# kisasexypantera94/hpfw

Hardware: AMD Instinct MI355X
Metric: hashprints/sec (index) + Hamming matches/sec (search), 30 s@44.1 kHz clips (higher is better)
Workload: dtype f32 (transforms, dB) + int8 digits / int64 sums (projection); 1 GPU; configs[1]: 1000 x 30 s synthetic 44.1 kHz PCM16 clips per GPU, hashprint extraction only (CQT + dB + projection + bit pack), inputs resident in HBM; clips_per_gpu=1000, hashprints_per_clip=2320, parallelism=clips sharded over 1 GPU(s), no collective on this path

## Files before the change

hpfw_amd/csrc/extract.hip:

```cpp
#include "handle.h"

int pass_clips(hpfw_gpu *h, const DevPlan *dp, int64_t n_clips)
{
    const hpfw::HostPlan &p = dp->hp;
    size_t per_clip = (size_t)121 * p.c * 4 + (size_t)64 * std::max(p.n_frames, 1) * 4;
    if (p.bluestein)
        per_clip += 2 * hpfw::bz_plane_bytes(dp->bz, 1) + (size_t)(p.kmax - p.kmin) * 8;
    else
        per_clip += (size_t)hpfw::z_floats_per_clip(p.hq, p.n2) * 4 + (size_t)p.n1 * p.q2w * 8;
    size_t work = 0;
    for (const hpfw::CqClassDev &cd : dp->cls) work = std::max(work, hpfw::cq_big_work_bytes(cd, 1));
    per_clip += work;
    const int64_t fit = std::max<int64_t>(1, (int64_t)(((size_t)24 << 30) / per_clip));
    const int64_t cap = std::min<int64_t>(h->batch, fit), n = std::max<int64_t>(n_clips, 1);
    const int64_t passes = (n + cap - 1) / cap;
    return (int)((n + passes - 1) / passes);
}

int ensure_ws(hpfw_gpu *h, const DevPlan *dp, int nb, int ns)
{
    const hpfw::HostPlan &p = dp->hp;
    size_t work = 0;
    for (const hpfw::CqClassDev &cd : dp->cls) work = std::max(work, hpfw::cq_big_work_bytes(cd, nb));
    if (work) {
        int rc = ensure(h->d_cqwork, work);
        if (rc) return rc;
    }
    const size_t planar = p.bluestein ? hpfw::bz_plane_bytes(dp->bz, nb) : 0;
    const size_t need[7] = {p.bluestein ? planar : (size_t)nb * hpfw::z_floats_per_clip(p.hq, p.n2) * 4,
                            p.bluestein ? (size_t)nb * (p.kmax - p.kmin) * 8 : (size_t)nb * p.n1 * p.q2w * 8,
                            (size_t)ns * 121 * p.c * 4, (size_t)ns * 64 * (size_t)std::max(p.n_frames, 1) * 4,
                            (size_t)ns * 121 * hpfw::kCqMaxWaves * 4,
                            0, planar};
    for (int i = 0; i < 7; ++i) {
        int rc = ensure(h->ws[i], need[i], h);
        if (rc) return rc;
    }
    return ensure(h->d_clipmax, (size_t)ns * 4, h);
}

namespace {
int ensure_side_streams(hpfw_gpu *h)
{
    if (h->cq_join[hpfw_gpu::kCqSide - 1]) return HPFW_OK;
    bool ok = h->cq_fork.create() == hipSuccess;
    for (int k = 0; k < hpfw_gpu::kCqSide && ok; ++k) ok = h->cq_side[k].create() == hipSuccess && h->cq_join[k].create() == hipSuccess;
    return ok ? HPFW_OK : fail(HPFW_E_HIP, "side streams");
}

class Fanout {
public:
    Fanout(hpfw_gpu *h, hipStream_t s) : h_(h), s_(s) {}
    Fanout(const Fanout &) = delete;
    Fanout &operator=(const Fanout &) = delete;
    ~Fanout()
    {
        for (int k = 0; k < hpfw_gpu::kCqSide; ++k) {
            if (!(used_ >> k & 1u)) continue;
            hipStream_t side = h_->cq_side[k].get();
            hipEvent_t join = h_->cq_join[k].get();
            if (report(h_, hipEventRecord(join, side), "side stream join") || report(h_, hipStreamWaitEvent(s_, join, 0), "side stream join"))
                (void)hipStreamSynchronize(side);
        }
    }
    int fork(int n)
    {
        int rc = ensure_side_streams(h_);
        if (rc) return rc;
        HIP_TRY(hipEventRecord(h_->cq_fork.get(), s_));
        for (int k = 0; k < n; ++k) HIP_TRY(hipStreamWaitEvent(h_->cq_side[k].get(), h_->cq_fork.get(), 0));
        return 0;
    }
    hipStream_t lane(int k)
    {
        if (k == 0) return s_;
        used_ |= 1u << (k - 1);
        return h_->cq_side[k - 1].get();
    }

private:
    hpfw_gpu *h_;
    hipStream_t s_;
    unsigned used_ = 0;
};

#if defined(HPFW_ROWS_SNAP) || defined(HPFW_ROWS_STAMPS)
hpfw::cf *g_rows_snap = nullptr;
#endif

int run_forward(hpfw_gpu *h, DevPlan *dp, const int16_t *d_pcm, int nb, hpfw::cf *x, hipStream_t s)
{
    const hpfw::HostPlan &p = dp->hp;
    float *yp = h->ws[0].as<float>();
    int rc;
    if (p.bluestein) {
        float *other = h->ws[6].as<float>();
        if (h->bz_chunk > 0 && nb >= 6 * h->bz_chunk) {
            const int lanes = h->fwd_streams;
            Fanout fan(h, s);
            if (lanes > 1 && (rc = fan.fork(lanes - 1))) return rc;
            const int64_t region = (int64_t)(hpfw::bz_plane_bytes(dp->bz, h->bz_chunk) / sizeof(float));
            int i = 0;
            for (int c0 = 0; c0 < nb; c0 += h->bz_chunk, ++i) {
                const int nc = std::min(nb - c0, h->bz_chunk);
                const int lane = i % lanes;
                hipStream_t st = fan.lane(lane);
                float *ya = yp + lane * region, *yb = other + lane * region;
                {
                    Timed t(h, K_COLS, st);
                    hpfw::launch_bz_cols_first(dp->bz, d_pcm + (int64_t)c0 * p.n, p.n, nc, ya, st);
                }
                {
                    Timed t(h, K_ROWS, st);
                    hpfw::launch_bz_rows_both(dp->rows, dp->bz, ya, nc, yb, st);
                }
                {
                    Timed t(h, K_COLS, st);
                    hpfw::launch_bz_cols_last(dp->bz, yb, nc, x + (int64_t)c0 * dp->cq.xclip, st);
                }
            }
            return check_launch("bz_chunks");
        }
        {
            Timed t(h, K_COLS, s);
            hpfw::launch_bz_cols_first(dp->bz, d_pcm, p.n, nb, yp, s);
        }
        if ((rc = check_launch("bz_cols"))) return rc;
        {
            Timed t(h, K_ROWS, s);
            hpfw::launch_bz_rows_both(dp->rows, dp->bz, yp, nb, other, s);
        }
        if ((rc = check_launch("bz_rows"))) return rc;
        {
            Timed t(h, K_COLS, s);
            hpfw::launch_bz_cols_last(dp->bz, other, nb, x, s);
        }
        return check_launch("bz_cols");
    }
    Timed span(h, K_FWD, s);
    hpfw::ColsQArgs cols = dp->cols;
    cols.variant = h->cols_variant;
    if (h->fwd_chunk > 0 && nb >= 6 * h->fwd_chunk) {
        const int lanes = h->fwd_streams;
        Fanout fan(h, s);
        if (lanes > 1 && (rc = fan.fork(lanes - 1))) return rc;
        const int64_t region = (int64_t)h->fwd_chunk * dp->rows_out.zclip;
        int i = 0;
        for (int c0 = 0; c0 < nb; c0 += h->fwd_chunk, ++i) {
            const int nc = std::min(nb - c0, h->fwd_chunk);
            const int lane = i % lanes;
            hipStream_t st = fan.lane(lane);
            float *zr = yp + lane * region;
            {
                Timed t(h, K_COLS, st);
                hpfw::launch_fwd_cols_q(cols, d_pcm + (int64_t)c0 * p.n, p.n, nc, zr, st);
            }
            {
                Timed t(h, K_ROWS, st);
                hpfw::launch_fwd_rows2(dp->rows, dp->rows_out, zr, nc, x + (int64_t)c0 * dp->rows_out.n1 * dp->rows_out.q2w, st);
            }
        }
        return check_launch("fwd_chunks");
    }
    {
        Timed t(h, K_COLS, s);
        hpfw::launch_fwd_cols_q(cols, d_pcm, p.n, nb, yp, s);
    }
    if ((rc = check_launch("fwd_cols"))) return rc;
    {
        Timed t(h, K_ROWS, s);
#if defined(HPFW_ROWS_SNAP)
        dp->rows.snap = g_rows_snap;
#endif
#if defined(HPFW_ROWS_STAMPS)
        dp->rows.stamps = reinterpret_cast<long long *>(g_rows_snap);
#endif
        hpfw::launch_fwd_rows2(dp->rows, dp->rows_out, yp, nb, x, s);
    }
    return check_launch("fwd_rows");
}
}

int run_front(hpfw_gpu *h, DevPlan *dp, const int16_t *d_pcm, int nb, int slot, bool finish_db, hipStream_t s)
{
    using hpfw::cf;
    const hpfw::HostPlan &p = dp->hp;
    cf *x = h->ws[1].as<cf>();
    float *mag = h->ws[2].as<float>() + (size_t)slot * 121 * p.c;
    float *mm = h->ws[4].as<float>() + (size_t)slot * 121 * hpfw::kCqMaxWaves;
    float *clipmax = h->d_clipmax.as<float>() + slot;
    int rc;
    if ((rc = run_forward(h, dp, d_pcm, nb, x, s))) return rc;
    {
        Timed t(h, K_CQ, s);
        int n_lds = 0;
        for (const hpfw::CqClassDev &cd : dp->cls) n_lds += cd.outer ? 0 : 1;
        const bool fork = h->cq_concurrent && n_lds > 1 && nb >= 4;
        Fanout fan(h, s);
        if (fork && (rc = fan.fork(hpfw_gpu::kCqSide))) return rc;
        int turn = 0;
        for (size_t ci = dp->cls.size(); ci-- > 0;) {
            const hpfw::CqClassDev &cd = dp->cls[ci];
            if (cd.outer) {
                hpfw::launch_cq_big_class(dp->cq, cd, x, nb, h->d_cqwork.as<cf>(), mag, mm, h->db_fast ? hpfw::kDbFast : hpfw::kDbSpec, s);
                continue;
            }
            const int lane = fork ? turn++ % (hpfw_gpu::kCqSide + 1) : 0;
            hpfw::launch_cq_class(dp->cq, cd, x, nb, mag, mm, h->db_fast ? hpfw::kDbFast : hpfw::kDbSpec, fan.lane(lane));
        }
        if ((rc = check_launch("cq_chirpz"))) return rc;
    }
    {
        Timed t(h, K_DB, s);
        hpfw::launch_clipmax(mm, clipmax, nb, s);
        if (finish_db) hpfw::launch_db_finish(mag, clipmax, nb, (int64_t)121 * p.c, s);
    }
    return check_launch("db");
}

namespace {
int run_back(hpfw_gpu *h, DevPlan *dp, const void *images, int n_shifts, int ns, uint64_t *d_hp, hipStream_t s)
{
    const hpfw::HostPlan &p = dp->hp;
    const float *sdb = h->ws[2].as<float>();
    int rc;
    if (h->projection) {
        {
            Timed t(h, K_PROJECT, s);
            hpfw::launch_hashprints_q(images, n_shifts, sdb, h->d_clipmax.as<float>(), ns, p.c, d_hp, nullptr, s);
        }
        return check_launch("project");
    }
    float *proj = h->ws[3].as<float>();
    {
        Timed t(h, K_PROJECT, s);
        hpfw::launch_project(h->d_fpack.as<float>(), sdb, h->d_clipmax.as<float>(), ns, p.c, proj, s);
    }
    if ((rc = check_launch("project"))) return rc;
    {
        Timed t(h, K_PACK, s);
        hpfw::launch_pack(proj, ns, p.n_frames, d_hp, s);
    }
    return check_launch("delta_pack");
}

constexpr int kBackBatch = 1024;

int check_filters(const hpfw_gpu *h) { return h->has_filters ? 0 : fail(HPFW_E_NOFILTERS, "no filters: call hpfw_gpu_set_filters or hpfw_gpu_learn_filters first"); }

int check_shifts(const int32_t *shifts, int n_shifts)
{
    if (!shifts || n_shifts < 1 || n_shifts > hpfw::kMaxShifts) return fail(HPFW_E_INVALID, "shifts: 1 to 64 values");
    for (int i = 0; i < n_shifts; ++i) {
        if (shifts[i] < -(hpfw::kBins - 1) || shifts[i] > hpfw::kBins - 1) return fail(HPFW_E_INVALID, "shifts: |s| <= 120");
        for (int j = 0; j < i; ++j)
            if (shifts[j] == shifts[i]) return fail(HPFW_E_INVALID, "shifts: values must be distinct");
    }
    return 0;
}

int shift_images(hpfw_gpu *h, const int32_t *shifts, int n_shifts, hipStream_t s)
{
    std::vector<int32_t> want(shifts, shifts + n_shifts);
    if (want == h->shift_images_of) return 0;
    h->shift_images_of.clear();
    int rc;
    if ((rc = ensure(h->d_shift_images, (size_t)n_shifts * hpfw::project_q_image_bytes()))) return rc;
    hpfw::ShiftList sl{n_shifts, {}};
    for (int i = 0; i < n_shifts; ++i) sl.s[i] = shifts[i];
    hpfw::launch_shift_filter_images(h->d_fq_image.get(), sl, h->d_shift_images.get(), s);
    if ((rc = check_launch("shift_filter_images"))) return rc;
    h->shift_images_of = std::move(want);
    return 0;
}

int check_transposed(hpfw_gpu *h, const int32_t *shifts, int n_shifts)
{
    int rc;
    if ((rc = check_shifts(shifts, n_shifts))) return rc;
    if (!h) return fail(HPFW_E_INVALID, "null handle");
    if (!h->projection) return fail(HPFW_E_INVALID, "transposed extraction needs projection mode 1 (fixed point)");
    if ((rc = check_filters(h))) return rc;
    return 0;
}

int hashprints_from_db(hpfw_gpu *h, const float *d_db, int64_t n_clips, int64_t c, const int32_t *shifts, int n_shifts, uint64_t *d_hp,
                       hipStream_t s)
{
    const int64_t nf = c - (hpfw::kCtx - 1), nhp = nf - hpfw::kLag;
    HIP_TRY(hipSetDevice(h->device));
    return ordered_call(h, s, [&] {
        int rc;
        if (n_shifts && (rc = shift_images(h, shifts, n_shifts, s))) return rc;
        const void *images = n_shifts ? h->d_shift_images.get() : h->d_fq_image.get();
        const int nbmax = 256;
        if (!h->projection && (rc = ensure(h->ws[3], (size_t)nbmax * 64 * (size_t)nf * 4))) return rc;
        for (int64_t c0 = 0; c0 < n_clips; c0 += nbmax) {
            const int nb = (int)std::min<int64_t>(nbmax, n_clips - c0);
            if (h->projection) {
                Timed t(h, K_PROJECT, s);
                hpfw::launch_hashprints_q(images, n_shifts, d_db + c0 * 121 * c, nullptr, nb, (int)c, d_hp + c0 * std::max(n_shifts, 1) * nhp,
                                          nullptr, s);
            } else {
                hpfw::launch_project(h->d_fpack.as<float>(), d_db + c0 * 121 * c, nullptr, nb, (int)c, h->ws[3].as<float>(), s);
                hpfw::launch_pack(h->ws[3].as<float>(), nb, (int)nf, d_hp + c0 * nhp, s);
            }
            if ((rc = check_launch("project"))) return rc;
        }
        return 0;
    });
}

constexpr size_t kTempoBudget = (size_t)256 << 20;

int check_tempos(const float *tempos, int n_tempos, int n_shifts)
{
    if (!tempos || n_tempos < 1 || n_tempos > hpfw::kMaxTempos) return fail(HPFW_E_INVALID, "tempos: 1 to 64 values");
    for (int i = 0; i < n_tempos; ++i) {
        if (!(tempos[i] >= 0.5f && tempos[i] <= 2.0f)) return fail(HPFW_E_INVALID, "tempos: finite values in [0.5, 2]");
        for (int j = 0; j < i; ++j)
            if (hpfw::tempo_step(tempos[j]) == hpfw::tempo_step(tempos[i]))
                return fail(HPFW_E_INVALID, "tempos: values must have distinct steps rint(65536 / tempo)");
    }
    if ((int64_t)n_tempos * std::max(n_shifts, 1) > hpfw::kMaxShifts) return fail(HPFW_E_INVALID, "tempos x shifts: at most 64 variants");
    return 0;
}

int check_tempo_call(hpfw_gpu *h, const float *tempos, int n_tempos, const int32_t *shifts, int n_shifts, hpfw::TempoList *tl)
{
    int rc;
    if ((rc = check_tempos(tempos, n_tempos, n_shifts))) return rc;
    if ((shifts || n_shifts) && (rc = check_shifts(shifts, n_shifts))) return rc;
    if (!h) return fail(HPFW_E_INVALID, "null handle");
    if (!h->projection) return fail(HPFW_E_INVALID, "tempo extraction needs projection mode 1 (fixed point)");
    if ((rc = check_filters(h))) return rc;
    tl->n = n_tempos;
    for (int i = 0; i < n_tempos; ++i) tl->step[i] = hpfw::tempo_step(tempos[i]);
    return 0;
}

int64_t tempo_common_columns(int64_t c, const hpfw::TempoList &tl)
{
    int64_t ct = INT64_MAX;
    for (int i = 0; i < tl.n; ++i) ct = std::min(ct, hpfw::tempo_columns(c, tl.step[i]));
    return ct;
}

int tempo_back(hpfw_gpu *h, const void *images, int n_shifts, const float *d_db, int64_t nb, int64_t c, const hpfw::TempoList &tl,
               int64_t ct, uint64_t *d_hp, hipStream_t s)
{
    const int64_t per_pair = (int64_t)std::max(n_shifts, 1) * (ct - (hpfw::kCtx - 1) - hpfw::kLag);
    const size_t pair_bytes = (size_t)hpfw::kBins * ct * 4;
    const int64_t pairs = std::max<int64_t>(1, (int64_t)(kTempoBudget / pair_bytes));
    const int64_t cb = pairs >= tl.n ? std::min<int64_t>(pairs / tl.n, nb) : 1;
    const int tb = pairs >= tl.n ? tl.n : (int)pairs;
    int rc;
    if ((rc = ensure(h->d_tempo, (size_t)cb * tb * pair_bytes, h))) return rc;
    float *scaled = h->d_tempo.as<float>();
    for (int64_t c0 = 0; c0 < nb; c0 += cb) {
        const int nc = (int)std::min(cb, nb - c0);
        for (int j0 = 0; j0 < tl.n; j0 += tb) {
            hpfw::TempoList sub{std::min(tb, tl.n - j0), {}};
            for (int j = 0; j < sub.n; ++j) sub.step[j] = tl.step[j0 + j];
            hpfw::launch_tempo_scale(d_db + c0 * hpfw::kBins * c, nc, c, sub, ct, scaled, s);
            if ((rc = check_launch("tempo_scale"))) return rc;
            {
                Timed t(h, K_PROJECT, s);
                hpfw::launch_hashprints_q(images, n_shifts, scaled, nullptr, nc * sub.n, (int)ct, d_hp + (c0 * tl.n + j0) * per_pair, nullptr, s);
            }
            if ((rc = check_launch("project"))) return rc;
        }
    }
    return 0;
}

int extract_tempo_pcm16(hpfw_gpu *h, const int16_t *d_pcm, int64_t n_samples, int64_t n_clips, const float *tempos, int n_tempos,
                        const int32_t *shifts, int n_shifts, uint64_t *d_hp, void *stream)
{
    hpfw::TempoList tl;
    int rc = check_tempo_call(h, tempos, n_tempos, shifts, n_shifts, &tl);
    if (rc) return rc;
    if (!d_pcm || !d_hp || n_clips < 0) return fail(HPFW_E_INVALID, "bad argument");
    HIP_TRY(hipSetDevice(h->device));
    DevPlan *dp;
    if ((rc = get_plan(h, n_samples, &dp))) return rc;
    const int64_t c = dp->hp.c, ct = tempo_common_columns(c, tl);
    if (ct - (hpfw::kCtx - 1) - hpfw::kLag < 1) return fail(HPFW_E_UNSUPPORTED, "clip too short to yield a hashprint at the slowest tempo");
    if (n_clips == 0) return 0;
    const int64_t per_clip = (int64_t)tl.n * std::max(n_shifts, 1) * (ct - (hpfw::kCtx - 1) - hpfw::kLag);
    hipStream_t s = (hipStream_t)stream;
    return ordered_call(h, s, [&] {
        if (n_shifts && (rc = shift_images(h, shifts, n_shifts, s))) return rc;
        const void *images = n_shifts ? h->d_shift_images.get() : h->d_fq_image.get();
        const int nbmax = pass_clips(h, dp, n_clips);
        if ((rc = ensure_ws(h, dp, nbmax, nbmax))) return rc;
        for (int64_t c0 = 0; c0 < n_clips; c0 += nbmax) {
            const int nb = (int)std::min<int64_t>(nbmax, n_clips - c0);
            if ((rc = run_front(h, dp, d_pcm + c0 * n_samples, nb, 0, true, s))) return rc;
            if ((rc = tempo_back(h, images, n_shifts, h->ws[2].as<float>(), nb, c, tl, ct, d_hp + c0 * per_clip, s))) return rc;
        }
        return 0;
    });
}

int extract_pcm16(hpfw_gpu *h, const int16_t *d_pcm, int64_t n_samples, int64_t n_clips, const int32_t *shifts, int n_shifts,
                  uint64_t *d_hp, void *stream)
{
    if (!h || !d_pcm || !d_hp || n_clips < 0) return fail(HPFW_E_INVALID, "bad argument");
    if (int rc = check_filters(h)) return rc;
    HIP_TRY(hipSetDevice(h->device));
    DevPlan *dp;
    int rc = get_plan(h, n_samples, &dp);
    if (rc) return rc;
    if (dp->hp.n_hp <= 0) return fail(HPFW_E_UNSUPPORTED, "clip too short to yield a hashprint");
    hipStream_t s = (hipStream_t)stream;
    return ordered_call(h, s, [&] {
        if (n_shifts && (rc = shift_images(h, shifts, n_shifts, s))) return rc;
        const void *images = n_shifts ? h->d_shift_images.get() : h->d_fq_image.get();
        const int nbmax = pass_clips(h, dp, n_clips);
        const int nsmax = (int)std::min<int64_t>(std::max(kBackBatch, nbmax), std::max<int64_t>(n_clips, 1));
        if ((rc = ensure_ws(h, dp, nbmax, nsmax))) return rc;
        for (int64_t s0 = 0; s0 < n_clips; s0 += nsmax) {
            const int ns = (int)std::min<int64_t>(nsmax, n_clips - s0);
            for (int c0 = 0; c0 < ns; c0 += nbmax) {
                const int nb = std::min(nbmax, ns - c0);
                if ((rc = run_front(h, dp, d_pcm + (s0 + c0) * n_samples, nb, c0, false, s))) return rc;
            }
            if ((rc = run_back(h, dp, images, n_shifts, ns, d_hp + s0 * std::max(n_shifts, 1) * dp->hp.n_hp, s))) return rc;
        }
        return 0;
    });
}

template <class Device>
int staged_pcm16_host(hpfw_gpu *h, const int16_t *pcm, int64_t n_samples, int64_t n_clips, int64_t per_clip, uint64_t *hp,
                      Device device)
{
    int rc;
    const int64_t chunk = std::min<int64_t>(n_clips, std::max<int64_t>(1, (192ll << 20) / (n_samples * 2)));
    if ((rc = ensure(h->stage_hp, (size_t)n_clips * std::max<int64_t>(per_clip, 1) * 8))) return rc;
    for (int b = 0; b < 2; ++b) {
        if (b == 1 && chunk >= n_clips) break;
        if ((rc = ensure(h->stage_pcm[b], (size_t)chunk * n_samples * 2))) return rc;
    }
    if (!h->stage_consumed[1]) {
        HIP_TRY(h->stage_copy.create());
        HIP_TRY(h->stage_comp.create());
        for (int b = 0; b < 2; ++b) {
            HIP_TRY(h->stage_copied[b].create());
            HIP_TRY(h->stage_consumed[b].create());
        }
    }
    hipStream_t s_copy = h->stage_copy.get(), s_comp = h->stage_comp.get();
    uint64_t *d_hp = h->stage_hp.as<uint64_t>();
    int64_t ci = 0;
    for (int64_t c0 = 0; !rc && c0 < n_clips; c0 += chunk, ++ci) {
        const int b = (int)(ci & 1);
        const int64_t cnt = std::min(chunk, n_clips - c0);
        int16_t *d_pcm = h->stage_pcm[b].as<int16_t>();
        hipEvent_t copied = h->stage_copied[b].get(), consumed = h->stage_consumed[b].get();
        if (ci >= 2 && hipStreamWaitEvent(s_copy, consumed, 0) != hipSuccess) rc = fail(HPFW_E_HIP, "event wait failed");
        if (!rc && hipMemcpyAsync(d_pcm, pcm + c0 * n_samples, (size_t)cnt * n_samples * 2, hipMemcpyHostToDevice, s_copy) !=
                       hipSuccess)
            rc = fail(HPFW_E_HIP, "H2D copy failed");
        if (!rc && (hipEventRecord(copied, s_copy) != hipSuccess || hipStreamWaitEvent(s_comp, copied, 0) != hipSuccess))
            rc = fail(HPFW_E_HIP, "event record failed");
        if (!rc) rc = device(d_pcm, cnt, d_hp + c0 * per_clip, s_comp);
        if (!rc && hipEventRecord(consumed, s_comp) != hipSuccess) rc = fail(HPFW_E_HIP, "event record failed");
    }
    if (hipStreamSynchronize(s_copy) != hipSuccess && !rc) rc = fail(HPFW_E_HIP, "H2D copy failed");
    if (!rc && hipMemcpyAsync(hp, d_hp, (size_t)n_clips * per_clip * 8, hipMemcpyDeviceToHost, s_comp) != hipSuccess)
        rc = fail(HPFW_E_HIP, "D2H copy failed");
    if (hipStreamSynchronize(s_comp) != hipSuccess && !rc) rc = fail(HPFW_E_HIP, "kernel execution failed");
    return rc;
}
}

extern "C" {

int hpfw_gpu_hashprints_from_db(hpfw_gpu *h, const float *d_db, int64_t n_clips, int64_t c, uint64_t *d_hp, void *stream)
{
    if (!h || !d_db || !d_hp) return fail(HPFW_E_INVALID, "null argument");
    if (int rc = check_filters(h)) return rc;
    if (c - (hpfw::kCtx - 1) - hpfw::kLag <= 0) return 0;
    return hashprints_from_db(h, d_db, n_clips, c, nullptr, 0, d_hp, (hipStream_t)stream);
}

int hpfw_gpu_stage_delta_q(hpfw_gpu *h, const float *d_db, int64_t n_clips, int64_t c, int64_t *d_delta, uint64_t *d_hp, void *stream)
{
    if (!h || !d_db || !d_delta) return fail(HPFW_E_INVALID, "null argument");
    if (int rc = check_filters(h)) return rc;
    const int64_t nhp = c - (hpfw::kCtx - 1) - hpfw::kLag;
    if (nhp <= 0 || n_clips <= 0) return 0;
    if (n_clips > 65535) return fail(HPFW_E_INVALID, "at most 65535 clips per call");
    HIP_TRY(hipSetDevice(h->device));
    hipStream_t s = (hipStream_t)stream;
    return ordered_call(h, s, [&] {
        uint64_t *hp = d_hp;
        if (!hp) {
            if (int rc = ensure(h->ws[3], (size_t)n_clips * (size_t)nhp * 8)) return rc;
            hp = h->ws[3].as<uint64_t>();
        }
        hpfw::launch_hashprints_q(h->d_fq_image.get(), 0, d_db, nullptr, (int)n_clips, (int)c, hp, (long long *)d_delta, s);
        return check_launch("project");
    });
}

int hpfw_gpu_hashprints_from_db_transposed(hpfw_gpu *h, const float *d_db, int64_t n_clips, int64_t c, const int32_t *shifts,
                                           int n_shifts, uint64_t *d_hp, void *stream)
{
// ... 448 lines not shown
```

hpfw_amd/csrc/handle.h:

```cpp
#pragma once
#include <hip/hip_runtime.h>

#include <algorithm>
#include <cstdio>
#include <cstdlib>
#include <cstring>
#include <condition_variable>
#include <chrono>
#include <map>
#include <memory>
#include <mutex>
#include <set>
#include <string>
#include <vector>

#include "../../include/hpfw_gpu.h"
#include "combiner.h"
#include "hip_owned.h"
#include "kernels.h"
#include "legacy_internal.h"
#include "plan.h"

using hpfw::DevBuf, hpfw::Event, hpfw::HostBuf, hpfw::Stream;

int fail(int code, const std::string &msg);

#define HIP_TRY(expr)                                                                                   \
    do {                                                                                                \
        hipError_t e_ = (expr);                                                                         \
        if (e_ != hipSuccess)                                                                           \
            return fail(HPFW_E_HIP, std::string(#expr) + ": " + hipGetErrorString(e_));                 \
    } while (0)

struct DevPlan {
    hpfw_gpu *owner = nullptr;
    std::vector<DevBuf> blocks;
    char *cur = nullptr;
    size_t left = 0;
    char *chunk_base = nullptr;
    std::vector<char> stage;
    std::vector<std::pair<size_t, size_t>> staged;
    hpfw::HostPlan hp;
    hpfw::ColsQArgs cols;
    hpfw::Rows2Out rows_out;
    hpfw::RowsArgs rows;
    hpfw::BzArgs bz;
    hpfw::CqPlanDev cq;
    std::vector<hpfw::CqClassDev> cls;
    size_t bytes = 0;
    uint64_t last_use = 0;
    ~DevPlan();
};

struct PlanTiming;

enum KernelKind { K_ROWS = 0, K_COLS, K_CQ, K_DB, K_PROJECT, K_PACK, K_SCAN, K_TOPK, K_PAIRS, K_FWD, K_COUNT };

struct TimedLaunch {
    int kind;
    Event a, b;
};

struct CallStatus {
    int rc = 0;
    std::string msg;
};

struct hpfw_gpu {
    int device = 0;
    bool has_filters = false;
    DevBuf d_fpack;
    DevBuf d_fq_image;
    int projection = 1;
    struct PlanCache {
        PlanCache();
        ~PlanCache();
        std::multimap<size_t, DevBuf> dev_pool;
        size_t dev_pool_bytes = 0;
        std::map<int64_t, std::unique_ptr<DevPlan>> plans;
        std::mutex host_mtx;
        std::condition_variable host_cv;
        std::map<int64_t, std::unique_ptr<hpfw::HostPlan>> host_ready;
        std::set<int64_t> host_seen;
        size_t plan_bytes = 0;
        uint64_t plan_clock = 0;
        uint64_t idle_clock = 0;
        std::unique_ptr<PlanTiming> plan_timing;
        Stream plan_stream;
        HostBuf pin_ring;
        size_t pin_off = 0;
        Event plan_ev;
        bool plan_ev_pending = false;
    } cache;
    unsigned conventions = 0;
    int batch = 256;
    DevBuf ws[7];
    struct Index {
        DevBuf d_db;
        std::vector<int64_t> db_off{0};
        DevBuf d_db_off;
        bool db_off_dirty = true;
        uint32_t clip_base = 0;
        DevBuf d_best, d_q_off;
        DevBuf d_qa;
        DevBuf d_gk;
        DevBuf d_topk_scratch;
        DevBuf d_shift_hits;
    } index;
    struct Learn {
        DevBuf d_cov;
        DevBuf d_cov_ws;
        DevBuf d_cov_tiles;
        int64_t cov_files = 0;
        std::map<std::vector<int>, DevBuf> cfg_fpack;
        DevBuf d_cfg_proj;
        struct CfgCov {
            DevBuf d_accum;
            DevBuf d_tiles;
            int64_t clips = 0;
        };
        std::map<std::vector<int>, CfgCov> cfg_cov;
        DevBuf d_cfg_cov_ws;
    } learn;
    struct Mel {
        bool ready = false;
        hpfw::HostPlan plan;
        hpfw::RowsArgs rows;
        const float *d_win = nullptr, *d_cpack = nullptr;
        std::vector<DevBuf> owned;
        DevBuf d_work, d_small;
    } mel;
    DevBuf d_cqwork;
    static constexpr int kCqSide = 4;
    Stream cq_side[kCqSide];
    Event cq_fork, cq_join[kCqSide];
    int cq_concurrent = 1;
    int fwd_chunk = 16, fwd_streams = 2;
    int cols_variant = 0;
    unsigned prune = 1;
    bool db_fast = true;
    int bz_chunk = 32;
    DevBuf stage_pcm[2];
    DevBuf stage_hp;
    Stream stage_copy, stage_comp;
    Event stage_copied[2], stage_consumed[2];
    DevBuf d_clipmax;
    Event order_ev;
    hipStream_t order_stream = nullptr;
    enum { kOrderNone, kOrderEvent, kOrderSync } order = kOrderNone;
    CallStatus call;
    Event ev0, ev1;
    unsigned timing_mask = 0;
    std::vector<TimedLaunch> timed;
    std::vector<std::pair<Event, Event>> ev_pool;
    float k_ms[K_COUNT] = {0};
    int k_launches[K_COUNT] = {0};
    std::unique_ptr<hpfw::Combiner> combiner;
    struct Resample {
        struct Table {
            int32_t L = 0, M = 0, T = 0;
            DevBuf d_taps;
        };
        std::map<int, Table> tables;
        DevBuf in, out;
    } rs;
    DevBuf d_shift_images;
    std::vector<int32_t> shift_images_of;
    DevBuf d_tempo;
    DevBuf d_windows;
};

int ensure(DevBuf &b, size_t need, hpfw_gpu *pool_owner = nullptr);

inline int report(hpfw_gpu *h, hipError_t e, const char *what)
{
    if (e != hipSuccess && !h->call.rc) h->call = {HPFW_E_HIP, std::string(what) + ": " + hipGetErrorString(e)};
    return e != hipSuccess;
}

template <class Body>
int ordered_call(hpfw_gpu *h, hipStream_t s, Body &&body)
{
    if (h->order_stream != s) {
        if (h->order == hpfw_gpu::kOrderEvent) HIP_TRY(hipStreamWaitEvent(s, h->order_ev.get(), 0));
        if (h->order == hpfw_gpu::kOrderSync) HIP_TRY(hipStreamSynchronize(h->order_stream));
    }
    if (h->cache.plan_ev_pending) {
        HIP_TRY(hipStreamWaitEvent(s, h->cache.plan_ev.get(), 0));
        h->cache.plan_ev_pending = false;
    }
    CallStatus outer = std::exchange(h->call, CallStatus{});
    int rc = body();
    const hipError_t recorded = hipEventRecord(h->order_ev.get(), s);
    h->order_stream = s;
    h->order = recorded == hipSuccess ? hpfw_gpu::kOrderEvent : hpfw_gpu::kOrderSync;
    CallStatus mine = std::exchange(h->call, std::move(outer));
    if (!rc && mine.rc) rc = fail(mine.rc, mine.msg);
    if (!rc && recorded != hipSuccess) rc = fail(HPFW_E_HIP, std::string("hipEventRecord: ") + hipGetErrorString(recorded));
    return rc;
}

struct Timed {
    hpfw_gpu *h;
    int kind;
    hipStream_t s;
    bool on = false;
    Event a, b;
    Timed(hpfw_gpu *h_, int kind_, hipStream_t s_) : h(h_), kind(kind_), s(s_)
    {
        if (!((h->timing_mask >> kind) & 1u)) return;
        if (h->ev_pool.empty()) {
            if (report(h, a.create(hipEventDefault), "timing event") || report(h, b.create(hipEventDefault), "timing event")) return;
        } else {
            a = std::move(h->ev_pool.back().first);
            b = std::move(h->ev_pool.back().second);
            h->ev_pool.pop_back();
        }
        on = !report(h, hipEventRecord(a.get(), s), "timing event record");
    }
    ~Timed()
    {
        if (on && !report(h, hipEventRecord(b.get(), s), "timing event record")) h->timed.push_back({kind, std::move(a), std::move(b)});
    }
};

inline int check_launch(const char *what)
{
    hipError_t e = hipGetLastError();
    if (e != hipSuccess) return fail(HPFW_E_HIP, std::string("launch of ") + what + ": " + hipGetErrorString(e));
    return 0;
}

struct HostTrip {
    int rc = 0;
    std::vector<std::pair<DevBuf, void *>> bufs;
    template <class T>
    T *take(size_t bytes, const void *src = nullptr, int fill = -1, void *dst = nullptr)
    {
        DevBuf &b = bufs.emplace_back(DevBuf(), dst).first;
        if (!rc && b.alloc(bytes) != hipSuccess) rc = fail(HPFW_E_NOMEM, "hipMalloc failed");
        if (!rc && ((src && hipMemcpy(b.get(), src, bytes, hipMemcpyHostToDevice) != hipSuccess) ||
                    (fill >= 0 && hipMemset(b.get(), fill, bytes) != hipSuccess)))
            rc = fail(HPFW_E_HIP, "H2D copy failed");
        return b.as<T>();
    }
    template <class Call>
    int run(bool wait, Call call)
    {
        if (!rc) rc = call();
        if (!rc && wait && hipDeviceSynchronize() != hipSuccess) rc = fail(HPFW_E_HIP, "kernel execution failed");
        for (auto &[b, dst] : bufs)
            if (!rc && dst && hipMemcpy(dst, b.get(), b.capacity(), hipMemcpyDeviceToHost) != hipSuccess) rc = fail(HPFW_E_HIP, "D2H copy failed");
        return rc;
    }
};

int get_plan(hpfw_gpu *h, int64_t n, DevPlan **out);
hipError_t init_plans(hpfw_gpu *h);
void clear_plans(hpfw_gpu *h);
int pass_clips(hpfw_gpu *h, const DevPlan *dp, int64_t n_clips);
int ensure_ws(hpfw_gpu *h, const DevPlan *dp, int nb, int ns);
int run_front(hpfw_gpu *h, DevPlan *dp, const int16_t *d_pcm, int nb, int slot, bool finish_db, hipStream_t s);
```

hpfw_amd/csrc/handle.hip:

```cpp
#include "handle.h"

namespace {
thread_local std::string g_err;

const char *const kKernelNames[K_COUNT] = {"fwd_rows", "fwd_cols", "cq_chirpz", "db",
                                           "project_mfma", "delta_pack", "hamming_scan", "topk", "pcm_pairs", "fwd_span"};
}

int fail(int code, const std::string &msg)
{
    g_err = msg;
    return code;
}

extern "C" {

const char *hpfw_gpu_last_error(void) { return g_err.c_str(); }
void hpfw_internal_set_error(const char *msg) { g_err = msg ? msg : ""; }
const char *hpfw_gpu_version(void) { return "hpfw-gpu 0.1 (gfx950)"; }

int hpfw_gpu_create(int device, hpfw_gpu **out)
{
    if (!out) return fail(HPFW_E_INVALID, "out is NULL");
    *out = nullptr;
    int n = 0;
    HIP_TRY(hipGetDeviceCount(&n));
    if (device < 0 || device >= n) return fail(HPFW_E_INVALID, "no such device");
    HIP_TRY(hipSetDevice(device));
    auto h = std::make_unique<hpfw_gpu>();
    h->device = device;
    if (std::getenv("HPFW_CQ_SERIAL")) h->cq_concurrent = 0;
    if (const char *e = std::getenv("HPFW_FWD_CHUNK")) h->fwd_chunk = std::max(0, atoi(e));
    if (const char *e = std::getenv("HPFW_BZ_CHUNK")) h->bz_chunk = std::max(0, atoi(e));
    if (const char *e = std::getenv("HPFW_COLS_VARIANT")) h->cols_variant = atoi(e);
    if (const char *e = std::getenv("HPFW_PRUNE")) h->prune = (unsigned)std::strtoul(e, nullptr, 0);
    if (const char *e = std::getenv("HPFW_DB_TERM")) h->db_fast = std::strcmp(e, "spec") != 0;
    if (const char *e = std::getenv("HPFW_FWD_STREAMS")) h->fwd_streams = std::min(hpfw_gpu::kCqSide + 1, std::max(1, atoi(e)));
    if (const char *e = std::getenv("HPFW_PROJECTION"))
        h->projection = std::strcmp(e, "f32") == 0 ? 0 : 1;
    if (h->ev0.create(hipEventDefault) != hipSuccess || h->ev1.create(hipEventDefault) != hipSuccess || h->order_ev.create() != hipSuccess ||
        init_plans(h.get()) != hipSuccess)
        return fail(HPFW_E_HIP, "hipEventCreate failed");
    *out = h.release();
    return 0;
}

int hpfw_gpu_device(const hpfw_gpu *h) { return h ? h->device : -1; }

void hpfw_gpu_destroy(hpfw_gpu *h)
{
    if (!h) return;
    (void)hipSetDevice(h->device);
    (void)hipDeviceSynchronize();
    delete h;
}

int hpfw_gpu_set_filters(hpfw_gpu *h, const float *f)
{
    if (!h || !f) return fail(HPFW_E_INVALID, "null argument");
    HIP_TRY(hipSetDevice(h->device));
    std::vector<float> packed((size_t)hpfw::kFilters * hpfw::kFrame);
    hpfw::pack_filters_for_mfma(f, packed.data());
    if (!h->d_fpack) HIP_TRY(h->d_fpack.alloc(packed.size() * 4));
    HIP_TRY(hipMemcpy(h->d_fpack.get(), packed.data(), packed.size() * 4, hipMemcpyHostToDevice));
    std::vector<int8_t> image;
    hpfw::pack_filters_q(f, image);
    if (!h->d_fq_image) HIP_TRY(h->d_fq_image.alloc(image.size()));
    HIP_TRY(hipMemcpy(h->d_fq_image.get(), image.data(), image.size(), hipMemcpyHostToDevice));
    h->shift_images_of.clear();
    h->has_filters = true;
    return 0;
}

int hpfw_gpu_set_projection(hpfw_gpu *h, int mode)
{
    if (!h || (mode != 0 && mode != 1)) return fail(HPFW_E_INVALID, "projection mode must be 0 (f32 chain) or 1 (fixed point)");
    h->projection = mode;
    return 0;
}

int hpfw_gpu_get_projection(hpfw_gpu *h) { return h ? h->projection : -1; }

int hpfw_gpu_set_conventions(hpfw_gpu *h, unsigned flags)
{
    if (!h || flags > hpfw::kConvAll) return fail(HPFW_E_INVALID, "unknown convention flag");
    HIP_TRY(hipSetDevice(h->device));
    if (flags != h->conventions) {
        HIP_TRY(hipDeviceSynchronize());
        clear_plans(h);
    }
    h->conventions = flags;
    return 0;
}

int hpfw_gpu_set_batch(hpfw_gpu *h, int clips)
{
    if (!h || clips < 0 || clips > 4096) return fail(HPFW_E_INVALID, "batch out of range");
    h->batch = clips == 0 ? 256 : clips;
    return 0;
}

int hpfw_gpu_timer_start(hpfw_gpu *h, void *stream)
{
    if (!h) return fail(HPFW_E_INVALID, "null handle");
    HIP_TRY(hipEventRecord(h->ev0.get(), (hipStream_t)stream));
    return 0;
}

int hpfw_gpu_timer_stop(hpfw_gpu *h, void *stream, float *ms)
{
    if (!h || !ms) return fail(HPFW_E_INVALID, "null argument");
    HIP_TRY(hipEventRecord(h->ev1.get(), (hipStream_t)stream));
    HIP_TRY(hipEventSynchronize(h->ev1.get()));
    HIP_TRY(hipEventElapsedTime(ms, h->ev0.get(), h->ev1.get()));
    return 0;
}

int hpfw_gpu_set_kernel_timing(hpfw_gpu *h, int mask)
{
    if (!h) return fail(HPFW_E_INVALID, "null handle");
    h->timing_mask = (unsigned)mask;
    for (TimedLaunch &t : h->timed) h->ev_pool.emplace_back(std::move(t.a), std::move(t.b));
    h->timed.clear();
    std::memset(h->k_ms, 0, sizeof(h->k_ms));
    std::memset(h->k_launches, 0, sizeof(h->k_launches));
    return 0;
}

int hpfw_gpu_get_kernel_timing(hpfw_gpu *h, const char **names, float *ms, int *launches, int *n)
{
    if (!h || !names || !ms || !launches || !n) return fail(HPFW_E_INVALID, "null argument");
    for (const TimedLaunch &t : h->timed) {
        HIP_TRY(hipEventSynchronize(t.b.get()));
        float e = 0.0f;
        HIP_TRY(hipEventElapsedTime(&e, t.a.get(), t.b.get()));
        h->k_ms[t.kind] += e;
        h->k_launches[t.kind] += 1;
    }
    for (TimedLaunch &t : h->timed) h->ev_pool.emplace_back(std::move(t.a), std::move(t.b));
    h->timed.clear();
    const int cap = *n;
    int w = 0;
    for (int i = 0; i < K_COUNT && w < cap; ++i, ++w) {
        names[w] = kKernelNames[i];
        ms[w] = h->k_ms[i];
        launches[w] = h->k_launches[i];
    }
    *n = w;
    return 0;
}

}
```

hpfw_amd/csrc/hip_owned.h:

```cpp
#pragma once
#include <cstddef>
#include <utility>

#include <hip/hip_runtime_api.h>

namespace hpfw {

struct DeviceMem {
    static hipError_t alloc(void **p, size_t bytes) { return hipMalloc(p, bytes); }
    static hipError_t release(void *p) { return hipFree(p); }
};
struct PinnedMem {
    static hipError_t alloc(void **p, size_t bytes) { return hipHostMalloc(p, bytes, hipHostMallocDefault); }
    static hipError_t release(void *p) { return hipHostFree(p); }
};

template <class Mem>
class Buffer {
public:
    Buffer() = default;
    Buffer(Buffer &&o) noexcept : p_(std::exchange(o.p_, nullptr)), cap_(std::exchange(o.cap_, 0)) {}
    Buffer &operator=(Buffer &&o) noexcept
    {
        std::swap(p_, o.p_);
        std::swap(cap_, o.cap_);
        return *this;
    }
    ~Buffer() { reset(); }

    hipError_t alloc(size_t bytes)
    {
        if (p_) {
            const hipError_t e = Mem::release(p_);
            p_ = nullptr;
            cap_ = 0;
            if (e != hipSuccess) return e;
        }
        const hipError_t e = Mem::alloc(&p_, bytes);
        if (e == hipSuccess) cap_ = bytes;
        else p_ = nullptr;
        return e;
    }
    hipError_t ensure(size_t bytes) { return cap_ >= bytes ? hipSuccess : alloc(bytes); }
    void reset()
    {
        if (p_) (void)Mem::release(p_);
        p_ = nullptr;
        cap_ = 0;
    }

    void *get() const { return p_; }
    template <class T>
    T *as() const { return static_cast<T *>(p_); }
    size_t capacity() const { return cap_; }
    explicit operator bool() const { return p_ != nullptr; }

private:
    void *p_ = nullptr;
    size_t cap_ = 0;
};

using DevBuf = Buffer<DeviceMem>;
using HostBuf = Buffer<PinnedMem>;

template <class H, hipError_t (*Destroy)(H)>
class Handle {
public:
    Handle() = default;
    Handle(Handle &&o) noexcept : h_(std::exchange(o.h_, nullptr)) {}
    Handle &operator=(Handle &&o) noexcept
    {
        std::swap(h_, o.h_);
        return *this;
    }
    ~Handle() { reset(); }
    void reset()
    {
        if (h_) (void)Destroy(h_);
        h_ = nullptr;
    }
    H get() const { return h_; }
    explicit operator bool() const { return h_ != nullptr; }

protected:
    template <class F>
    hipError_t make(F &&create)
    {
        reset();
        const hipError_t e = create(&h_);
        if (e != hipSuccess) h_ = nullptr;
        return e;
    }

private:
    H h_ = nullptr;
};

class Stream : public Handle<hipStream_t, hipStreamDestroy> {
public:
    hipError_t create()
    {
        return make([](hipStream_t *s) { return hipStreamCreateWithFlags(s, hipStreamNonBlocking); });
    }
};

class Event : public Handle<hipEvent_t, hipEventDestroy> {
public:
    hipError_t create(unsigned flags = hipEventDisableTiming)
    {
        return make([flags](hipEvent_t *e) { return hipEventCreateWithFlags(e, flags); });
    }
};

}
```

Baseline: 262.7 million hashprints/s.

## Cost-balance CQ class launches across lanes capped by hardware queue count

Replaces the round-robin assignment of LDS CQ classes to side streams with a greedy longest-first plan. Classes are sorted by transform size, and each one goes to the lane with the least accumulated estimated cost, using a fitted per-size weight table. The lane count is capped by GPU_MAX_HW_QUEUES (default 4, giving 3 lanes) so streams do not oversubscribe hardware queues. An optional mode gives the first side streams high priority. The goal is less tail imbalance in the concurrent CQ phase. The tradeoffs are a hard-coded cost model and possibly fewer lanes than before.

```diff
diff --git a/hpfw_amd/csrc/cq_launch_plan.h b/hpfw_amd/csrc/cq_launch_plan.h
--- /dev/null
+++ b/hpfw_amd/csrc/cq_launch_plan.h
@@ -0,0 +1,64 @@
+#pragma once
+#include <cstdint>
+#include <cstdlib>
+#include <vector>
+
+namespace hpfw {
+
+struct CqPlanClass {
+    int p;
+    int n_bands;
+};
+
+struct CqLaunch {
+    int cls;
+    int lane;
+};
+
+inline int64_t cq_class_weight(int p)
+{
+    constexpr int kN = 5;
+    constexpr int kP[kN] = {3072, 4096, 6144, 8192, 12288};
+    constexpr int64_t kW[kN] = {27798 / 5, 31468 / 4, 36684 / 3, 36326 / 2, 39108 / 1};
+    if (p <= kP[0]) return kW[0] * p / kP[0];
+    if (p >= kP[kN - 1]) return kW[kN - 1] * p / kP[kN - 1];
+    int i = 1;
+    while (kP[i] < p) ++i;
+    return kW[i - 1] + (kW[i] - kW[i - 1]) * (p - kP[i - 1]) / (kP[i] - kP[i - 1]);
+}
+
+inline std::vector<CqLaunch> cq_launch_plan(const std::vector<CqPlanClass> &classes, int64_t n_clips, int max_lanes)
+{
+    const int n = (int)classes.size(), lanes = max_lanes < 1 ? 1 : max_lanes;
+    std::vector<CqLaunch> plan(n);
+    for (int i = 0; i < n; ++i) plan[i].cls = i;
+    for (int i = 1; i < n; ++i)
+        for (int k = i; k > 0 && classes[plan[k - 1].cls].p < classes[plan[k].cls].p; --k) {
+            const CqLaunch t = plan[k];
+            plan[k] = plan[k - 1];
+            plan[k - 1] = t;
+        }
+    std::vector<int64_t> cost(lanes, 0);
+    for (CqLaunch &l : plan) {
+        int best = lanes > 1 ? 1 : 0;
+        for (int k = 2; k <= lanes; ++k)
+            if (cost[k % lanes] < cost[best]) best = k % lanes;
+        l.lane = best;
+        const CqPlanClass &c = classes[l.cls];
+        cost[best] += (int64_t)c.n_bands * (n_clips < 1 ? 1 : n_clips) * cq_class_weight(c.p);
+    }
+    return plan;
+}
+
+inline int cq_hw_queues(const char *env)
+{
+    if (!env || !*env) return 4;
+    char *end = nullptr;
+    const long q = std::strtol(env, &end, 10);
+    if (end == env || *end) return 4;
+    return q < 2 ? 2 : q > 32 ? 32 : (int)q;
+}
+
+inline int cq_default_lanes(int side_streams, int hw_queues) { return side_streams + 1 < hw_queues - 1 ? side_streams + 1 : hw_queues - 1; }
+
+}
diff --git a/hpfw_amd/csrc/extract.hip b/hpfw_amd/csrc/extract.hip
--- a/hpfw_amd/csrc/extract.hip
+++ b/hpfw_amd/csrc/extract.hip
@@ -1,4 +1,6 @@
 #include "handle.h"
+
+#include "cq_launch_plan.h"
 
 int pass_clips(hpfw_gpu *h, const DevPlan *dp, int64_t n_clips)
 {
@@ -44,7 +46,19 @@
 {
     if (h->cq_join[hpfw_gpu::kCqSide - 1]) return HPFW_OK;
     bool ok = h->cq_fork.create() == hipSuccess;
-    for (int k = 0; k < hpfw_gpu::kCqSide && ok; ++k) ok = h->cq_side[k].create() == hipSuccess && h->cq_join[k].create() == hipSuccess;
+    int least = 0, greatest = 0;
+    bool ranked = false;
+    if (h->cq_plan == 2) {
+        if (hipDeviceGetStreamPriorityRange(&least, &greatest) == hipSuccess) ranked = greatest < least;
+        else (void)hipGetLastError();
+    }
+    for (int k = 0; k < hpfw_gpu::kCqSide && ok; ++k) {
+        if (!(ranked && k < 2 && k < h->cq_lanes - 1 && h->cq_side[k].create_with_priority(greatest) == hipSuccess)) {
+            (void)hipGetLastError();
+            ok = h->cq_side[k].create() == hipSuccess;
+        }
+        ok = ok && h->cq_join[k].create() == hipSuccess;
+    }
     return ok ? HPFW_OK : fail(HPFW_E_HIP, "side streams");
 }
 
@@ -193,11 +207,15 @@
     if ((rc = run_forward(h, dp, d_pcm, nb, x, s))) return rc;
     {
         Timed t(h, K_CQ, s);
-        int n_lds = 0;
-        for (const hpfw::CqClassDev &cd : dp->cls) n_lds += cd.outer ? 0 : 1;
-        const bool fork = h->cq_concurrent && n_lds > 1 && nb >= 4;
+        std::vector<hpfw::CqPlanClass> lds;
+        for (size_t ci = dp->cls.size(); ci-- > 0;)
+            if (!dp->cls[ci].outer) lds.push_back({dp->cls[ci].p, dp->cls[ci].n_bands});
+        const bool fork = h->cq_concurrent && lds.size() > 1 && nb >= 4;
+        const int lanes = !fork ? 1 : h->cq_plan ? h->cq_lanes : hpfw_gpu::kCqSide + 1;
+        std::vector<hpfw::CqLaunch> plan;
+        if (h->cq_plan) plan = hpfw::cq_launch_plan(lds, nb, lanes);
         Fanout fan(h, s);
-        if (fork && (rc = fan.fork(hpfw_gpu::kCqSide))) return rc;
+        if (lanes > 1 && (rc = fan.fork(lanes - 1))) return rc;
         int turn = 0;
         for (size_t ci = dp->cls.size(); ci-- > 0;) {
             const hpfw::CqClassDev &cd = dp->cls[ci];
@@ -205,7 +223,8 @@
                 hpfw::launch_cq_big_class(dp->cq, cd, x, nb, h->d_cqwork.as<cf>(), mag, mm, h->db_fast ? hpfw::kDbFast : hpfw::kDbSpec, s);
                 continue;
             }
-            const int lane = fork ? turn++ % (hpfw_gpu::kCqSide + 1) : 0;
+            const int lane = h->cq_plan ? plan[turn].lane : turn % lanes;
+            ++turn;
             hpfw::launch_cq_class(dp->cq, cd, x, nb, mag, mm, h->db_fast ? hpfw::kDbFast : hpfw::kDbSpec, fan.lane(lane));
         }
         if ((rc = check_launch("cq_chirpz"))) return rc;
diff --git a/hpfw_amd/csrc/handle.h b/hpfw_amd/csrc/handle.h
--- a/hpfw_amd/csrc/handle.h
+++ b/hpfw_amd/csrc/handle.h
@@ -135,6 +135,8 @@
     Stream cq_side[kCqSide];
     Event cq_fork, cq_join[kCqSide];
     int cq_concurrent = 1;
+    int cq_plan = 1;
+    int cq_lanes = 3;
     int fwd_chunk = 16, fwd_streams = 2;
     int cols_variant = 0;
     unsigned prune = 1;
diff --git a/hpfw_amd/csrc/handle.hip b/hpfw_amd/csrc/handle.hip
--- a/hpfw_amd/csrc/handle.hip
+++ b/hpfw_amd/csrc/handle.hip
@@ -1,4 +1,6 @@
 #include "handle.h"
+
+#include "cq_launch_plan.h"
 
 namespace {
 thread_local std::string g_err;
@@ -30,6 +32,9 @@
     auto h = std::make_unique<hpfw_gpu>();
     h->device = device;
     if (std::getenv("HPFW_CQ_SERIAL")) h->cq_concurrent = 0;
+    if (const char *e = std::getenv("HPFW_CQ_PLAN"))
+        if ((e[0] == '0' || e[0] == '1' || e[0] == '2') && !e[1]) h->cq_plan = e[0] - '0';
+    h->cq_lanes = hpfw::cq_default_lanes(hpfw_gpu::kCqSide, hpfw::cq_hw_queues(std::getenv("GPU_MAX_HW_QUEUES")));
     if (const char *e = std::getenv("HPFW_FWD_CHUNK")) h->fwd_chunk = std::max(0, atoi(e));
     if (const char *e = std::getenv("HPFW_BZ_CHUNK")) h->bz_chunk = std::max(0, atoi(e));
     if (const char *e = std::getenv("HPFW_COLS_VARIANT")) h->cols_variant = atoi(e);
diff --git a/hpfw_amd/csrc/hip_owned.h b/hpfw_amd/csrc/hip_owned.h
--- a/hpfw_amd/csrc/hip_owned.h
+++ b/hpfw_amd/csrc/hip_owned.h
@@ -102,6 +102,10 @@
     {
         return make([](hipStream_t *s) { return hipStreamCreateWithFlags(s, hipStreamNonBlocking); });
     }
+    hipError_t create_with_priority(int priority)
+    {
+        return make([priority](hipStream_t *s) { return hipStreamCreateWithPriority(s, hipStreamNonBlocking, priority); });
+    }
 };
 
 class Event : public Handle<hipEvent_t, hipEventDestroy> {
```

Result: no change. 264.2 million hashprints/s, median of 5 (+0.6%).
